# Krabbens/edge-diffusion-tts

Measured on AMD Instinct MI355X. Metric: mel-frames/sec (whole node), 4-step DDIM, hidden=160 L=4, B=256 T=512, higher is better.
Workload: dtype f32

## Files before the change

### edge-diffusion-tts_amd/csrc/edtts_bf16.h

```cpp
typedef __bf16 bf8 __attribute__((ext_vector_type(8)));
typedef __bf16 bf2 __attribute__((ext_vector_type(2)));
typedef float f2v __attribute__((ext_vector_type(2)));

#define EDTTS_MFMA16(a, b, c) __builtin_amdgcn_mfma_f32_16x16x32_bf16((a), (b), (c), 0, 0, 0)

#ifndef EDTTS_STAMP_HEAD
#define EDTTS_STAMP_HEAD 0
#endif
#ifdef EDTTS_STAMPS
#ifndef EDTTS_STAMP_THREAD
#define EDTTS_STAMP_THREAD 0
#endif
#define STAMP16(i) do { if (a.stamps && blockIdx.x == 0 && threadIdx.x == EDTTS_STAMP_THREAD) a.stamps[i] = __builtin_amdgcn_s_memtime(); } while (0)
#define STAMPX16(p, i) do { if ((p) && blockIdx.x == 0 && threadIdx.x == EDTTS_STAMP_THREAD) (p)[i] = __builtin_amdgcn_s_memtime(); } while (0)
#else
#define STAMP16(i) do { } while (0)
#define STAMPX16(p, i) do { } while (0)
#endif

namespace edtts16 {
using namespace edtts;

template <int H_, int HEADS_, int MEL_, int NF_ = 2>
struct Cfg16 {
// ... 627 lines not shown
#pragma unroll
        for (int ft = 0; ft < NF; ++ft) v[ft] = gt[ft] = splat(0.f);
        gemm16_pair<C::KT, false>(ring, hn, v, gt);
        const f4 vb = *reinterpret_cast<const f4*>(params + 32 * j + 4 * g), gb = *reinterpret_cast<const f4*>(params + 32 * j + 16 + 4 * g);
#pragma unroll
        for (int ft = 0; ft < NF; ++ft) {
          v[ft] += vb;
          gt[ft] += gb;
          const f4 e = {fast_exp2(gt[ft][0] * -1.4426950408889634f), fast_exp2(gt[ft][1] * -1.4426950408889634f),
                        fast_exp2(gt[ft][2] * -1.4426950408889634f), fast_exp2(gt[ft][3] * -1.4426950408889634f)};
          const f4 d = e + 1.0f;
          const f4 rc = {__builtin_amdgcn_rcpf(d[0]), __builtin_amdgcn_rcpf(d[1]), __builtin_amdgcn_rcpf(d[2]), __builtin_amdgcn_rcpf(d[3])};
          act[u][ft] = (v[ft] * gt[ft]) * rc;
        }
      }
      bf8 ab[NF];
#pragma unroll
      for (int ft = 0; ft < NF; ++ft) ab[ft] = pack8(act[0][ft], act[1][ft]);
      ktile16<C::HT>(ring, ab, h);
    }
  }
  STAMP16(4);
  if (TAIL == TAIL_QKV) {
    if (valid) {
#pragma unroll
      for (int nt = 0; nt < C::HT; ++nt)
#pragma unroll
        for (int ft = 0; ft < NF; ++ft) stg4(a.h + h_at<C>(tile0, lane, nt, ft), h[nt][ft]);
    }
    bf8 hn[C::KT][NF];
    rms_norm_pack<C>(h, a.n1w, a.cond + (size_t)b * a.cond_bstride + ((size_t)(a.layer + 1) * 2) * 2 * C::H, g, hn);
    qkv_tail16<C>(ring, hn, a, b, m0, lane, valid);
  } else {
    bf8 hn[C::KT][NF];
    layer_norm_pack<C>(h, a.fnw, a.fnb, g, hn);
    for (int p = 0; p < C::MTP; ++p) {
      f4 e[2][NF];
#pragma unroll
      for (int ft = 0; ft < NF; ++ft) e[0][ft] = e[1][ft] = splat(0.f);
      gemm16_pair<C::KT, false>(ring, hn, e[0], e[1]);
#pragma unroll
      for (int u = 0; u < 2; ++u) {
        const int nt = 2 * p + u;
        if (nt >= C::MT) continue;
        const f4 ob = *reinterpret_cast<const f4*>(params + C::UPB_FLOATS + 16 * nt + 4 * g);
#pragma unroll
        for (int ft = 0; ft < NF; ++ft) {
          const int f = m0 + 16 * ft + fq;
          if (f >= a.T || !valid) continue;
          tail_store<TAIL>(a, f, Tb, ((size_t)b * a.T + f) * C::MEL + 16 * nt + 4 * g, e[u][ft] + ob);
        }
      }
    }
  }
  STAMP16(5);
  ring.drain();
  STAMP16(6);
}

}
```

### edge-diffusion-tts_amd/csrc/edtts_coop.h

```cpp
namespace edtts {

template <class C, int W>
struct Coop {
  static constexpr int NF = C::NF, HT = C::HT;
  static constexpr int TILES = 1;
  static constexpr int THREADS = 64 * W;
  static constexpr int O_BYTES = C::HEADS * C::OHEAD_BYTES;
  static constexpr int Q_BYTES = C::WF * C::H * 4;
  static constexpr int ACT_TILES = 2 * HT;
  static constexpr int ACT_BYTES = ACT_TILES * NF * 1024;
  static constexpr int A_BYTES = O_BYTES + Q_BYTES > ACT_BYTES ? O_BYTES + Q_BYTES : ACT_BYTES;
  static constexpr int X_BYTES = HT * NF * 1024;
  static constexpr int TILE_BYTES = A_BYTES + X_BYTES;
  static constexpr int LDS_BYTES = TILES * TILE_BYTES;
  static constexpr bool FITS = LDS_BYTES * (4 / W) <= 160 * 1024;
  static_assert(W == 2 || W == 4, "waves per tile");
};

template <int LK, bool TWO, class FA, class FB>
EDTTS_DEV void co_preload(__amdgpu_buffer_rsrc_t rs, unsigned voff, FA&& fa, FB&& fb, f4 (&ra)[LK], f4 (&rb)[LK]) {
#pragma unroll
  for (int i = 0; i < LK; ++i) {
    ra[i] = bufld4(rs, voff, fa(i));
    if (TWO) rb[i] = bufld4(rs, voff, fb(i));
// ... 251 lines not shown
            if (nt >= HT) continue;
            for (int k = 0; k < nj; ++k) {
              f4 ra[1], rb[1];
              auto one = [&](int) { return (F_FFN + (unsigned)(j0 + k) * 3u * HT + 2u * HT + (unsigned)nt) * 1024u; };
              co_preload<1, false>(rs, voff, one, one, ra, rb);
              co_ktiles<1, NF, 1, false, false>(rs, voff, ra, rb, one, one, one, one, [&](int, int ft) { return act[(k * NF + ft) * 64]; }, NrFull{}, dacc[i], dummy);
            }
          }
        }
      }
    }
#pragma unroll
    for (int i = 0; i < MINE; ++i)
      if (wv + i * W < HT) x_put(wv + i * W, dacc[i]);
  }
  if (TAIL == TAIL_QKV) {
    auto fr = [&](int t, int k) { return (f_tail + (unsigned)((t >> 1) * 2 * HT + 2 * k + (t & 1))) * 1024u; };
    CoGemm<HT, NF, W> gm;
    gm.preload(rs, voff, wv, 3 * HT, fr);
    __syncthreads();
    add_branch();
    if (valid) {
#pragma unroll
      for (int nt = 0; nt < HT; ++nt)
        if (nt % W == wv) {
#pragma unroll
          for (int ft = 0; ft < NF; ++ft) stg4(hp + 16 * nt + (size_t)ft * 16 * H, h[nt][ft]);
        }
    }
    const float* mod = a.cond + (size_t)b * a.cond_bstride + ((size_t)(a.layer + 1) * 2) * 2 * H;
    rms_norm_tile<HT, NF>(h, a.n1w, mod, g, h);
    coop_qkv<C, W>(a, rs, voff, gm, fr, h, wv, lane, b, m0, valid);
  } else {
    __syncthreads();
    add_branch();
    f4 hn[HT][NF];
    layer_norm_tile<HT, NF>(h, a.fnw, a.fnb, g, hn);
    for (int nt = wv; nt < C::MT; nt += W) {
      f4 e[NF], o[NF];
#pragma unroll
      for (int ft = 0; ft < NF; ++ft) e[ft] = o[ft] = splat(0.f);
      f4 fr[HT];
#pragma unroll
      for (int k = 0; k < HT; ++k) fr[k] = bufld4(rs, voff, (f_tail + (unsigned)(nt * HT + k)) * 1024u);
#pragma unroll
      for (int k = 0; k < HT; ++k)
#pragma unroll
        for (int r = 0; r < 4; ++r)
#pragma unroll
          for (int ft = 0; ft < NF; ++ft) {
            if (k & 1) o[ft] = EDTTS_MFMA(fr[k][r], hn[k][ft][r], o[ft]);
            else e[ft] = EDTTS_MFMA(fr[k][r], hn[k][ft][r], e[ft]);
          }
      const f4 ob = ldg4(a.outp_b + 16 * nt + 4 * g);
#pragma unroll
      for (int ft = 0; ft < NF; ++ft) {
        e[ft] += o[ft];
        const int f = m0 + 16 * ft + fq;
        if (!valid || f >= a.T) continue;
        const size_t idx = ((size_t)b * a.T + f) * C::MEL + 16 * nt + 4 * g;
        tail_store<TAIL>(a, f, Tb, idx, e[ft] + ob);
      }
    }
  }
}

template <class C, int TAIL, int W>
__global__ __launch_bounds__(64 * W) void k_layer_co(KArgs a) {
  extern __shared__ __attribute__((aligned(16))) char smem_co[];
  using CO = Coop<C, W>;
  static_assert(CO::FITS, "cooperative tile state must fit the CU's LDS");
  const int lane = threadIdx.x & 63;
  const int wave = __builtin_amdgcn_readfirstlane(threadIdx.x >> 6);
  const int tpu = a.Tp / C::WF, ntiles = a.B * tpu;
  int tile = remap_block(blockIdx.x, gridDim.x) * CO::TILES + wave / W;
  const bool valid = tile < ntiles;
  tile = valid ? tile : ntiles - 1;
  const int b = tile / tpu;
  coop_layer_tile<C, TAIL, W>(a, smem_co + (wave / W) * CO::TILE_BYTES, wave % W, lane, b, (tile - b * tpu) * C::WF, valid);
}

template <class C, int W>
__global__ __launch_bounds__(64 * W) void k_prologue_co(KArgs a) {
  extern __shared__ __attribute__((aligned(16))) char smem_co[];
  constexpr int NF = C::NF, HT = C::HT, MT = C::MT, H = C::H;
  const int lane = threadIdx.x & 63, fq = lane & 15, g = lane >> 4;
  const int wv = __builtin_amdgcn_readfirstlane(threadIdx.x >> 6);
  const int tpu = a.Tp / C::WF, ntiles = a.B * tpu;
  int tile = remap_block(blockIdx.x, gridDim.x);
  const bool valid = tile < ntiles;
  tile = valid ? tile : ntiles - 1;
  const int b = tile / tpu, m0 = (tile - b * tpu) * C::WF;
  const int Tb = utt_len(a.t_len, b, a.T, a.t_dbl);
  f4* const xb = reinterpret_cast<f4*>(smem_co) + lane;
  const __amdgpu_buffer_rsrc_t rs = make_rsrc(a.stream);
  const unsigned voff = (unsigned)lane * 16u;
// ... 43 lines not shown
```

### edge-diffusion-tts_amd/csrc/edtts_generic.h

```cpp
namespace edtts_gen {

enum { EPI_BIAS = 0, EPI_PE = 1, EPI_RESID = 2, EPI_SWIGLU = 3 };

struct GemmArgs {
  const float* X;
  const float* W;
  const float* bias;
  float* Y;
  const float* pe;
  int M, N, K, ldx, ldy, T;
  int vec_x, vec_w, vec_y;
  DropArgs dr;
};
constexpr int kGBM = 64, kGBN = 64, kGBK = 16, kGLd = kGBK + 1;

template <int EPI, bool DROP = false>
__global__ __launch_bounds__(256) void k_gen_gemm(GemmArgs a) {
  __shared__ float xs[kGBM][kGLd];
  __shared__ float ws[kGBN][kGLd];
  const int tid = threadIdx.x, lane = tid & 63, w = tid >> 6, fq = lane & 15, g = lane >> 4;
  const int m0 = blockIdx.x * kGBM;
  const int n0 = blockIdx.y * (EPI == EPI_SWIGLU ? kGBN / 2 : kGBN);
  const int lr = tid >> 2, lk = 4 * (tid & 3);
  int wrow;
// ... 303 lines not shown
    if (a.x0_all) a.x0_all[idx] = v0;
    a.x_prev[idx] = vn;
  } else if (TAIL == TAIL_VLMS) {
    const float v = a.v_uncond ? cfg_combine(e, a.v_uncond[idx], a.vp.cfg) : e;
    const float hn = a.lms.mode >= 2 ? a.h_new[idx] : 0.f, ho = a.lms.mode >= 3 ? a.h_old[idx] : 0.f;
    float v0, vn;
    lms_elem(a.x[idx], v, hn, ho, a.lms, v0, vn);
    a.x0_hist[idx] = v0;
    if (a.x0_all) a.x0_all[idx] = v0;
    if (a.known != nullptr) {
      const size_t row = (size_t)a.T * a.inj_mel, b = idx / row, r = idx - b * row, per = (size_t)a.inj_frames * a.inj_mel;
      if (r < per) {
        const size_t ki = b * per + r;
        vn = a.known[ki];
        if (a.p_coef2 != 0.f) {
          const float nz = a.noise ? a.noise[ki]
                                   : (a.seeds ? philox_normal4(a.seeds[b], a.step, r >> 2)[(int)(r & 3)] : philox_normal4(a.seed, a.step, ki >> 2)[(int)(ki & 3)]);
          vn = qsample_elem(vn, a.p_coef1, nz, a.p_coef2);
        }
      }
    }
    a.x_prev[idx] = vn;
  } else if (TAIL == TAIL_VPRED) {
    const float v = a.v_uncond ? cfg_combine(e, a.v_uncond[idx], a.vp.cfg) : e;
    a.x_prev[idx] = vpred_elem(a.x[idx], v, a.vp);
  } else if (TAIL == TAIL_DDPM) {
    const unsigned long long ge = a.philox_base + idx;
    const float nz = a.noise ? a.noise[idx] : philox_normal4(a.seed, a.step, ge >> 2)[(int)(ge & 3)];
    const DdpmCoef cf{a.p_coef1, a.p_coef2, a.p_sd};
    a.x_prev[idx] = ddpm_elem(a.x[idx], e, nz, cf);
  } else {
    float v0, vp;
    ddim_elem(a.x[idx], e, a.c_s1m, a.c_sab, a.c_sabp, a.c_dir, v0, vp);
    a.x0[idx] = v0;
    a.x_prev[idx] = vp;
  }
}
template <int TAIL>
EDTTS_DEV void tail_zero_elem(const KArgs& a, size_t idx) {
  if (TAIL == TAIL_LMS || TAIL == TAIL_VLMS) {
    a.x0_hist[idx] = 0.f;
    if (a.x0_all) a.x0_all[idx] = 0.f;
  } else if (TAIL == TAIL_DDIM) {
    a.x0[idx] = 0.f;
  }
  a.x_prev[idx] = 0.f;
}
EDTTS_DEV bool past_len(const int64_t* t_len, bool dbl, size_t idx, int T, int MEL) {
  if (t_len == nullptr) return false;
  const size_t row = idx / MEL;
  return (int)(row % T) >= utt_len_lane(t_len, (int)(row / T), T, dbl);
}
template <int TAIL>
__global__ __launch_bounds__(256) void k_gen_tail(KArgs a, const float* eps, size_t n, int vec, int MEL) {
  const size_t stride = (size_t)gridDim.x * blockDim.x;
  if (vec) {
    for (size_t i = (size_t)blockIdx.x * blockDim.x + threadIdx.x; i < n / 4; i += stride) {
      if constexpr (TAIL == TAIL_VLMS) {
        const size_t row = 4 * i / MEL;
        const int f = (int)(row % a.T);
        const int Tb = a.t_len ? utt_len_of(a.t_len[row / a.T], a.T, a.t_dbl) : a.T;
        tail_store<TAIL>(a, f, Tb, 4 * i, ldg4(eps + 4 * i));
        continue;
      }
      if (past_len(a.t_len, a.t_dbl, 4 * i, a.T, MEL)) tail_zero<TAIL>(a, 4 * i);
      else tail_apply<TAIL>(a, 4 * i, ldg4(eps + 4 * i));
    }
  } else {
    for (size_t i = (size_t)blockIdx.x * blockDim.x + threadIdx.x; i < n; i += stride) {
      if (past_len(a.t_len, a.t_dbl, i, a.T, MEL)) tail_zero_elem<TAIL>(a, i);
      else tail_elem<TAIL>(a, i, eps[i]);
    }
  }
}
__global__ __launch_bounds__(256) void k_gen_zero_past(float* y, const int64_t* t_len, int dbl, size_t n, int T, int MEL) {
  for (size_t i = (size_t)blockIdx.x * blockDim.x + threadIdx.x; i < n; i += (size_t)gridDim.x * blockDim.x)
    if (past_len(t_len, dbl, i, T, MEL)) y[i] = 0.f;
// ... 278 lines not shown
```

### edge-diffusion-tts_amd/csrc/edtts_kernels.hip

```cpp
#include <hip/hip_runtime.h>
#include <math.h>
#include <stdarg.h>
#include <stdlib.h>
#include <stdio.h>
#include <string.h>
#include <atomic>
#include <initializer_list>
#include <mutex>
#include <vector>

#include "../../include/edtts.h"
#include "edtts_device.h"

using namespace edtts;

static thread_local char g_err[512] = "";
static int fail(int code, const char* fmt, ...) __attribute__((format(printf, 2, 3)));
static int fail(int code, const char* fmt, ...) {
  va_list ap;
  va_start(ap, fmt);
  vsnprintf(g_err, sizeof(g_err), fmt, ap);
  va_end(ap);
  return code;
}
// ... 579 lines not shown
        for (int r = 0; r < 4; ++r) {
#pragma unroll
          for (int ft = 0; ft < NF; ++ft) h[nt][ft] = EDTTS_MFMA(fa[r], xin[kt][ft][r], h[nt][ft]);
#pragma unroll
          for (int ft = 0; ft < NF; ++ft) h[nt + 1][ft] = EDTTS_MFMA(fb[r], xin[kt][ft][r], h[nt + 1][ft]);
        }
        ring.template refill_after<N>(i);
        ring.template refill_after<N>(i + 1);
      }
    ring.advance(N);
  }
#pragma unroll
  for (int ft = 0; ft < NF; ++ft) {
    int f = m0 + 16 * ft + fq;
    f = f < a.max_pos ? f : a.max_pos - 1;
#pragma unroll
    for (int nt = 0; nt < C::HT; ++nt) h[nt][ft] += ldg4(a.pe + (size_t)f * C::H + 16 * nt + 4 * g);
  }
  {
    float* hp = a.h + ((size_t)b * a.Tp + m0 + fq) * C::H + 4 * g;
#pragma unroll
    for (int nt = 0; nt < C::HT; ++nt)
#pragma unroll
      for (int ft = 0; ft < NF; ++ft) stg4(hp + 16 * nt + (size_t)ft * 16 * C::H, h[nt][ft]);
  }
  f4 hn[C::HT][NF];
  const float* mod = a.cond + (size_t)b * a.cond_bstride;
  rms_norm_tile<C::HT, NF>(h, a.n1w, mod, g, hn);
  qkv_tail<C>(ring, hn, a, b, m0, lane);
}

enum { TAIL_QKV = 0, TAIL_EPS = 1, TAIL_DDIM = 2, TAIL_DDPM = 3, TAIL_LMS = 4, TAIL_VPRED = 5, TAIL_VLMS = 6 };

template <int TAIL>
EDTTS_DEV void tail_apply(const KArgs& a, size_t idx, f4 ev, bool blend = false) {
  if (TAIL == TAIL_EPS) {
    stg4(a.eps + idx, ev);
  } else if (TAIL == TAIL_LMS) {
    const f4 xv = ldg4(a.x + idx);
    f4 hn = splat(0.f), ho = splat(0.f);
    if (a.lms.mode >= 2) hn = ldg4(a.h_new + idx);
    if (a.lms.mode >= 3) ho = ldg4(a.h_old + idx);
    f4 x0, xn;
#pragma unroll
    for (int r = 0; r < 4; ++r) {
      float v0, vn;
      lms_elem(xv[r], ev[r], hn[r], ho[r], a.lms, v0, vn);
      x0[r] = v0;
      xn[r] = vn;
    }
    stg4(a.x0_hist + idx, x0);
    if (a.x0_all) stg4(a.x0_all + idx, x0);
    stg4(a.x_prev + idx, xn);
  } else if (TAIL == TAIL_VLMS) {
    const bool guided = a.v_uncond != nullptr;
    const f4 xv = ldg4(a.x + idx);
    const f4 vu = ldg4((guided ? a.v_uncond : a.x) + idx);
    f4 hn = splat(0.f), ho = splat(0.f);
    if (a.lms.mode >= 2) hn = ldg4(a.h_new + idx);
    if (a.lms.mode >= 3) ho = ldg4(a.h_old + idx);
    f4 x0, xn;
#pragma unroll
    for (int r = 0; r < 4; ++r) {
      const float v = guided ? cfg_combine(ev[r], vu[r], a.vp.cfg) : ev[r];
      float v0, vn;
      lms_elem(xv[r], v, hn[r], ho[r], a.lms, v0, vn);
      x0[r] = v0;
      xn[r] = vn;
    }
    stg4(a.x0_hist + idx, x0);
    if (a.x0_all) stg4(a.x0_all + idx, x0);
    if (!blend) stg4(a.x_prev + idx, xn);
  } else if (TAIL == TAIL_VPRED) {
    const bool guided = a.v_uncond != nullptr;
    const f4 xv = ldg4(a.x + idx);
    const f4 vu = ldg4((guided ? a.v_uncond : a.x) + idx);
    f4 v, xn;
#pragma unroll
    for (int r = 0; r < 4; ++r) v[r] = guided ? cfg_combine(ev[r], vu[r], a.vp.cfg) : ev[r];
#pragma unroll
    for (int r = 0; r < 4; ++r) xn[r] = vpred_elem(xv[r], v[r], a.vp);
    stg4(a.x_prev + idx, xn);
  } else if (TAIL == TAIL_DDPM) {
    const f4 xv = ldg4(a.x + idx);
    const f4 nz = a.noise ? ldg4(a.noise + idx) : philox_normal4(a.seed, a.step, (a.philox_base + idx) >> 2);
    const DdpmCoef cf{a.p_coef1, a.p_coef2, a.p_sd};
    f4 xp;
#pragma unroll
    for (int r = 0; r < 4; ++r) xp[r] = ddpm_elem(xv[r], ev[r], nz[r], cf);
    stg4(a.x_prev + idx, xp);
  } else {
    const f4 xv = ldg4(a.x + idx);
    f4 x0, xp;
#pragma unroll
    for (int r = 0; r < 4; ++r) {
      float v0, vp;
      ddim_elem(xv[r], ev[r], a.c_s1m, a.c_sab, a.c_sabp, a.c_dir, v0, vp);
      x0[r] = v0;
      xp[r] = vp;
    }
    stg4(a.x0 + idx, x0);
    stg4(a.x_prev + idx, xp);
  }
}
template <int TAIL>
EDTTS_DEV void tail_zero(const KArgs& a, size_t idx) {
  const f4 z = splat(0.f);
  if (TAIL == TAIL_EPS) {
    stg4(a.eps + idx, z);
  } else if (TAIL == TAIL_LMS || TAIL == TAIL_VLMS) {
    stg4(a.x0_hist + idx, z);
    if (a.x0_all) stg4(a.x0_all + idx, z);
    stg4(a.x_prev + idx, z);
  } else if (TAIL == TAIL_DDIM) {
    stg4(a.x0 + idx, z);
    stg4(a.x_prev + idx, z);
  } else {
    stg4(a.x_prev + idx, z);
  }
}
EDTTS_DEV void vlms_blend(const KArgs& a, size_t idx) {
  const size_t row = (size_t)a.T * a.inj_mel, b = idx / row, r = idx - b * row;
  const size_t ki = b * ((size_t)a.inj_frames * a.inj_mel) + r;
  const f4 kv = ldg4(a.known + ki);
  f4 o = kv;
  if (a.p_coef2 != 0.f) {
    const unsigned long long sd = a.seeds ? a.seeds[b] : a.seed;
    const f4 nz = a.noise ? ldg4(a.noise + ki) : philox_normal4(sd, a.step, (a.seeds ? r : ki) >> 2);
#pragma unroll
    for (int e = 0; e < 4; ++e) o[e] = qsample_elem(kv[e], a.p_coef1, nz[e], a.p_coef2);
  }
  stg4(a.x_prev + idx, o);
}
template <int TAIL>
EDTTS_DEV void tail_store(const KArgs& a, int f, int Tb, size_t idx, f4 ev) {
  if constexpr (TAIL == TAIL_VLMS) {
    const bool blend = a.known != nullptr && f < Tb && f < a.inj_frames;
    if (f < Tb) tail_apply<TAIL>(a, idx, ev, blend);
    else tail_zero<TAIL>(a, idx);
    if (blend) vlms_blend(a, idx);
  } else {
    if (f < Tb) tail_apply<TAIL>(a, idx, ev);
    else tail_zero<TAIL>(a, idx);
  }
}

struct QGlobal {
  __amdgpu_buffer_rsrc_t rs;
  unsigned v4, v2;
  int H;
  EDTTS_DEV QGlobal(const float* row_m0, int H_, int fq, int g) : rs(make_rsrc(row_m0)), v4((unsigned)(fq * H_ + 4 * g) * 4u), v2((unsigned)(fq * H_ + 2 * g) * 4u), H(H_) {}
  EDTTS_DEV f4 q4(int ft, int col) const { return bufld4(rs, v4, (unsigned)(ft * 16 * H + col) * 4u); }
  EDTTS_DEV f2 q2(int ft, int col) const { return bufld2(rs, v2, (unsigned)(ft * 16 * H + col) * 4u); }
};
struct QLds {
  const float* b4;
  const float* b2;
  int ld;
  EDTTS_DEV QLds(const float* tile, int ld_, int fq, int g) : b4(tile + fq * ld_ + 4 * g), b2(tile + fq * ld_ + 2 * g), ld(ld_) {}
  EDTTS_DEV f4 q4(int ft, int col) const { return *reinterpret_cast<const f4*>(b4 + ft * 16 * ld + col); }
  EDTTS_DEV f2 q2(int ft, int col) const { return *reinterpret_cast<const f2*>(b2 + ft * 16 * ld + col); }
};

template <class C, int TAIL>
EDTTS_DEV void layer_tile(const KArgs& a, float* smem, int wave, int lane, int b, int m0, int Tb, int Sb) {
  constexpr int NF = C::NF;
  const int fq = lane & 15, g = lane >> 4;
  f4* const stash = reinterpret_cast<f4*>(smem) + (size_t)wave * C::HT * NF * 64 + lane;
  constexpr int QLDS = C::H;
  float* qtile = smem + (size_t)C::WAVES * C::HT * NF * 256 + (size_t)wave * C::WF * QLDS;
  const size_t rowbase = (size_t)b * a.Tp + m0 + fq;

  STAMPX(a.stamps, 0, a.diag_skip);
  WStream<C> ring;
  ring.prime(a.stream, lane);

  f4 h[C::HT][NF];
// ... 78 lines not shown
#pragma unroll
    for (int nt = 0; nt < C::HT; ++nt) {
      const f4 db = ldg4(a.down_b + 16 * nt + 4 * g);
#pragma unroll
      for (int ft = 0; ft < NF; ++ft) h[nt][ft] = db;
    }
    for (int j = 0; j < a.ffn_tiles; ++j) {
      const f4 vb = ldg4(a.up_b + 32 * j + 4 * g), gb = ldg4(a.up_b + 32 * j + 16 + 4 * g);
      f4 v[NF], gt[NF], act[NF];
#pragma unroll
      for (int ft = 0; ft < NF; ++ft) v[ft] = gt[ft] = splat(0.f);
      gemm_phase_pair<C::HT>(ring, hn, v, gt);
      __builtin_amdgcn_sched_barrier(0);
#pragma unroll
      for (int ft = 0; ft < NF; ++ft) act[ft] = swiglu_tile(v[ft], gt[ft], vb, gb);
      __builtin_amdgcn_sched_barrier(0);
      ktile_phase<C::HT>(ring, act, h);
    }
    add_parked_h();
    STAMPX(a.stamps, 4, a.diag_skip);
  }
  if (TAIL == TAIL_QKV) {
    {
      float* hp = a.h + rowbase * C::H + 4 * g;
#pragma unroll
      for (int nt = 0; nt < C::HT; ++nt)
#pragma unroll
        for (int ft = 0; ft < NF; ++ft) stg4(hp + 16 * nt + (size_t)ft * 16 * C::H, h[nt][ft]);
    }
    const float* mod = a.cond + (size_t)b * a.cond_bstride + ((size_t)(a.layer + 1) * 2) * 2 * C::H;
    rms_norm_tile<C::HT, NF>(h, a.n1w, mod, g, h);
    qkv_tail<C>(ring, h, a, b, m0, lane);
  } else {
    f4 hn[C::HT][NF];
    layer_norm_tile<C::HT, NF>(h, a.fnw, a.fnb, g, hn);
#pragma unroll
    for (int nt = 0; nt < C::MT; ++nt) {
      const f4 ob = ldg4(a.outp_b + 16 * nt + 4 * g);
      f4 e[NF];
#pragma unroll
      for (int ft = 0; ft < NF; ++ft) e[ft] = splat(0.f);
      gemm_phase<C::HT>(ring, hn, e);
#pragma unroll
      for (int ft = 0; ft < NF; ++ft) {
        const int f = m0 + 16 * ft + fq;
        if (f >= a.T) continue;
        const size_t idx = ((size_t)b * a.T + f) * C::MEL + 16 * nt + 4 * g;
        tail_store<TAIL>(a, f, Tb, idx, e[ft] + ob);
      }
    }
  }
  STAMPX(a.stamps, 5, a.diag_skip);
#ifdef EDTTS_STAMPS
  asm volatile("s_waitcnt vmcnt(0)" ::: "memory");
#endif
  STAMPX(a.stamps, 6, a.diag_skip);
}

template <class C, int TAIL>
EDTTS_DEV void tail_zero_tile(const KArgs& a, int b, int m0, int lane) {
  const int fq = lane & 15, g = lane >> 4;
#pragma unroll
  for (int ft = 0; ft < C::NF; ++ft) {
    const int f = m0 + 16 * ft + fq;
    if (f >= a.T) continue;
#pragma unroll
    for (int nt = 0; nt < C::MT; ++nt) tail_zero<TAIL>(a, ((size_t)b * a.T + f) * C::MEL + 16 * nt + 4 * g);
  }
}
template <class C, int TAIL>
__global__ __launch_bounds__(C::THREADS, 1) void k_layer(KArgs a) {
  extern __shared__ __attribute__((aligned(16))) float smem[];
  const int lane = threadIdx.x & 63;
  const int wave = __builtin_amdgcn_readfirstlane(threadIdx.x >> 6);
  const TileId tl = wave_tile(a.B, a.Tp, C::WAVES, C::WF);
  if (!tl.valid) return;
  const int Tb = utt_len(a.t_len, tl.b, a.T, a.t_dbl);
  if (tl.m0 >= live_end(Tb)) {
    if constexpr (TAIL != TAIL_QKV) tail_zero_tile<C, TAIL>(a, tl.b, tl.m0, lane);
    return;
  }
  const int Sb = utt_len(a.s_len, tl.b, a.S);
// ... 1929 lines not shown
```

### edge-diffusion-tts_amd/csrc/edtts_samplers.h

```cpp

struct StepArgs {
  const float *alphas, *alpha_bar, *betas, *post_var;
  int n_table;
  const float *x, *eps, *noise;
  const int64_t *t, *t_prev;
  size_t n_per_batch;
  float eta;
  float *x_prev, *x0;
  int vec4;
};
static int step_vec4(size_t n_per_batch, std::initializer_list<const void*> ptrs) {
  uintptr_t m = 0;
  for (const void* p : ptrs) m |= (uintptr_t)p;
  return (n_per_batch & 3) == 0 && (m & 15) == 0;
}
EDTTS_DEV long clamp_idx(long v, int n) { return v < 0 ? 0 : (v >= n ? n - 1 : v); }

__global__ __launch_bounds__(256) void k_ddim(StepArgs a) {
  const int b = blockIdx.y;
  const float ab = a.alpha_bar[clamp_idx((long)a.t[b], a.n_table)];
  const long tp = (long)a.t_prev[b];
  const float abp = tp >= 0 ? a.alpha_bar[clamp_idx(tp, a.n_table)] : 1.0f;
  const DdimCoef cf = ddim_coef(ab, abp, a.eta);
  const float s1m = cf.s1m, sab = cf.sab, sabp = cf.sabp, cdir = cf.cdir, sigma = cf.sigma;
// ... 240 lines not shown

static unsigned step_blocks(const StepArgs& a) {
  const size_t bx = ((a.vec4 ? a.n_per_batch / 4 : a.n_per_batch) + 255) / 256;
  return bx > 2048 ? 2048u : (bx < 1 ? 1u : (unsigned)bx);
}

extern "C" {

int edtts_generate(const EdttsDims* dims, const void* packed, void* workspace, int B, int S, const int64_t* sem_idx,
                   const float* x_T, int num_steps, const int64_t* timesteps_host, const float* coef_host, float* x_work,
                   float* x0_out, void* stream) {
  return edtts_generate_len(dims, packed, workspace, B, S, sem_idx, nullptr, x_T, num_steps, timesteps_host, coef_host, x_work, x0_out,
                            stream);
}

int edtts_generate_len(const EdttsDims* dims, const void* packed, void* workspace, int B, int S, const int64_t* sem_idx,
                       const int64_t* s_len, const float* x_T, int num_steps, const int64_t* timesteps_host, const float* coef_host,
                       float* x_work, float* x0_out, void* stream) {
  const SettingsScope settings;
  Layout lo;
  TRY_G(make_layout(dims, &lo));
  if (!packed || !workspace || !sem_idx || !x_T || !timesteps_host || !coef_host || !x_work || !x0_out)
    return fail(EDTTS_ERR_ARG, "NULL pointer argument");
  if (num_steps < 1 || num_steps > lo.NSTEP)
    return fail(EDTTS_ERR_ARG, "num_steps=%d outside [1,%d] (step_emb rows; the reference raises IndexError)", num_steps, lo.NSTEP);
  const int T = 2 * S;
  TRY_G(check_shapes(lo, B, T, S));
  SamplerInputs in;
  in.t_host = timesteps_host; in.sem_idx = sem_idx;
  in.ln = Lens{s_len, s_len, true};
  in.x_T = x_T; in.x = x_work;
  return run_sampler(dims, lo, packed, workspace, B, T, S, num_steps, in, stream, [&](int i, int, size_t o) {
    StepTail tail;
    tail.kind = TAIL_DDIM; tail.x_prev = x_work + o; tail.x0 = x0_out + o; tail.coef = coef_host + 4 * i;
    return tail;
  });
}

int edtts_sample_multistep(const EdttsDims* dims, const void* packed, void* workspace, int B, int T, int S, const int64_t* sem_idx,
                           const float* sem_features, const float* x_T, int num_steps, const int64_t* timesteps_host,
                           const float* coef_host, float* hist, float* x0_all, float* x_out, void* stream) {
  return edtts_sample_multistep_len(dims, packed, workspace, B, T, S, sem_idx, sem_features, nullptr, nullptr, x_T, num_steps,
                                    timesteps_host, coef_host, hist, x0_all, x_out, stream);
}

int edtts_sample_multistep_len(const EdttsDims* dims, const void* packed, void* workspace, int B, int T, int S, const int64_t* sem_idx,
                               const float* sem_features, const int64_t* t_len, const int64_t* s_len, const float* x_T, int num_steps,
                               const int64_t* timesteps_host, const float* coef_host, float* hist, float* x0_all, float* x_out,
                               void* stream) {
  const SettingsScope settings;
  Layout lo;
  TRY_G(make_layout(dims, &lo));
  if (!sem_idx && !sem_features) return fail(EDTTS_ERR_ARG, "Either sem_idx or sem_features must be provided");
  if (!packed || !workspace || !x_T || !timesteps_host || !coef_host || !hist || !x_out) return fail(EDTTS_ERR_ARG, "NULL pointer argument");
  if (num_steps < 1 || num_steps > lo.NSTEP)
    return fail(EDTTS_ERR_ARG, "num_steps=%d outside [1,%d] (step_emb rows; the reference raises IndexError)", num_steps, lo.NSTEP);
  TRY_G(check_shapes(lo, B, T, S));
  TRY_G(check_lms_modes(coef_host, num_steps));
  SamplerInputs in;
  in.t_host = timesteps_host; in.sem_idx = sem_idx; in.sem_features = sem_features;
  in.ln = Lens{t_len, s_len};
  in.x_T = x_T; in.x = x_out;
  const size_t per = (size_t)B * T * lo.MEL;
  return run_sampler(dims, lo, packed, workspace, B, T, S, num_steps, in, stream, [&](int i, int, size_t o) {
    StepTail tail;
    tail.kind = TAIL_LMS; tail.x_prev = x_out + o;
    tail.lms = lms_step_args(coef_host + 8 * i, hist, x0_all, per, i, o);
// ... 177 lines not shown
```

Baseline: 8.746 million.

## Prefetch sampler-tail operands before output GEMM and skip intermediate x0 stores

Splits the fused sampler tail into request/update/commit phases, so loads of x, history, noise and bias for the output projection are issued before the final GEMM and their latency overlaps the MFMA work. Output tiles are grouped by a register-budget heuristic, and stores are batched after all updates. Separately, DDIM generation now writes x0 only on the last step, removing redundant global stores on earlier steps. This raises register pressure and adds scheduling barriers, which could lower occupancy or force spills.

New measurement: 8.723 million. About the same (-0.3%).

```diff
diff --git a/edge-diffusion-tts_amd/csrc/edtts_bf16.h b/edge-diffusion-tts_amd/csrc/edtts_bf16.h
--- a/edge-diffusion-tts_amd/csrc/edtts_bf16.h
+++ b/edge-diffusion-tts_amd/csrc/edtts_bf16.h
@@ -683,25 +683,24 @@
     rms_norm_pack<C>(h, a.n1w, a.cond + (size_t)b * a.cond_bstride + ((size_t)(a.layer + 1) * 2) * 2 * C::H, g, hn);
     qkv_tail16<C>(ring, hn, a, b, m0, lane, valid);
   } else {
+    constexpr int GP = tile_tail_group<NF, TAIL, C::KT * NF * 4, C::MTP, 2>();
+    TileTail<C, TAIL, 2 * GP> tt;
     bf8 hn[C::KT][NF];
     layer_norm_pack<C>(h, a.fnw, a.fnb, g, hn);
-    for (int p = 0; p < C::MTP; ++p) {
-      f4 e[2][NF];
-#pragma unroll
-      for (int ft = 0; ft < NF; ++ft) e[0][ft] = e[1][ft] = splat(0.f);
-      gemm16_pair<C::KT, false>(ring, hn, e[0], e[1]);
-#pragma unroll
-      for (int u = 0; u < 2; ++u) {
-        const int nt = 2 * p + u;
-        if (nt >= C::MT) continue;
-        const f4 ob = *reinterpret_cast<const f4*>(params + C::UPB_FLOATS + 16 * nt + 4 * g);
-#pragma unroll
-        for (int ft = 0; ft < NF; ++ft) {
-          const int f = m0 + 16 * ft + fq;
-          if (f >= a.T || !valid) continue;
-          tail_store<TAIL>(a, f, Tb, ((size_t)b * a.T + f) * C::MEL + 16 * nt + 4 * g, e[u][ft] + ob);
-        }
-      }
+    __builtin_amdgcn_sched_barrier(0);
+    tt.request(a, params + C::UPB_FLOATS, b, m0, Tb, lane, [](int i) { return i < C::MT ? i : -1; });
+#pragma unroll
+    for (int p0 = 0; p0 < C::MTP; p0 += GP) {
+      auto nt_of = [p0](int i) { return 2 * p0 + i < C::MT ? 2 * p0 + i : -1; };
+      if (p0 > 0) tt.request(a, params + C::UPB_FLOATS, b, m0, Tb, lane, nt_of);
+      f4 e[2 * GP][NF];
+#pragma unroll
+      for (int j = 0; j < GP; ++j) {
+#pragma unroll
+        for (int ft = 0; ft < NF; ++ft) e[2 * j][ft] = e[2 * j + 1][ft] = splat(0.f);
+        if (p0 + j < C::MTP) gemm16_pair<C::KT, false>(ring, hn, e[2 * j], e[2 * j + 1]);
+      }
+      tt.finish(a, b, m0, Tb, lane, nt_of, e, valid);
     }
   }
   STAMP16(5);
diff --git a/edge-diffusion-tts_amd/csrc/edtts_coop.h b/edge-diffusion-tts_amd/csrc/edtts_coop.h
--- a/edge-diffusion-tts_amd/csrc/edtts_coop.h
+++ b/edge-diffusion-tts_amd/csrc/edtts_coop.h
@@ -307,14 +307,23 @@
     rms_norm_tile<HT, NF>(h, a.n1w, mod, g, h);
     coop_qkv<C, W>(a, rs, voff, gm, fr, h, wv, lane, b, m0, valid);
   } else {
+    constexpr int MINE = (C::MT + W - 1) / W;
+    auto nt_of = [wv](int i) { return wv + i * W < C::MT ? wv + i * W : -1; };
+    TileTail<C, TAIL, MINE> tt;
     __syncthreads();
     add_branch();
     f4 hn[HT][NF];
     layer_norm_tile<HT, NF>(h, a.fnw, a.fnb, g, hn);
-    for (int nt = wv; nt < C::MT; nt += W) {
+    __builtin_amdgcn_sched_barrier(0);
+    tt.request(a, a.outp_b, b, m0, Tb, lane, nt_of);
+    f4 ev[MINE][NF];
+#pragma unroll
+    for (int i = 0; i < MINE; ++i) {
+      const int nt = nt_of(i);
       f4 e[NF], o[NF];
 #pragma unroll
-      for (int ft = 0; ft < NF; ++ft) e[ft] = o[ft] = splat(0.f);
+      for (int ft = 0; ft < NF; ++ft) ev[i][ft] = e[ft] = o[ft] = splat(0.f);
+      if (nt < 0) continue;
       f4 fr[HT];
 #pragma unroll
       for (int k = 0; k < HT; ++k) fr[k] = bufld4(rs, voff, (f_tail + (unsigned)(nt * HT + k)) * 1024u);
@@ -327,16 +336,10 @@
             if (k & 1) o[ft] = EDTTS_MFMA(fr[k][r], hn[k][ft][r], o[ft]);
             else e[ft] = EDTTS_MFMA(fr[k][r], hn[k][ft][r], e[ft]);
           }
-      const f4 ob = ldg4(a.outp_b + 16 * nt + 4 * g);
-#pragma unroll
-      for (int ft = 0; ft < NF; ++ft) {
-        e[ft] += o[ft];
-        const int f = m0 + 16 * ft + fq;
-        if (!valid || f >= a.T) continue;
-        const size_t idx = ((size_t)b * a.T + f) * C::MEL + 16 * nt + 4 * g;
-        tail_store<TAIL>(a, f, Tb, idx, e[ft] + ob);
-      }
-    }
+#pragma unroll
+      for (int ft = 0; ft < NF; ++ft) ev[i][ft] = e[ft] + o[ft];
+    }
+    tt.finish(a, b, m0, Tb, lane, nt_of, ev, valid);
   }
 }
 
diff --git a/edge-diffusion-tts_amd/csrc/edtts_generic.h b/edge-diffusion-tts_amd/csrc/edtts_generic.h
--- a/edge-diffusion-tts_amd/csrc/edtts_generic.h
+++ b/edge-diffusion-tts_amd/csrc/edtts_generic.h
@@ -359,7 +359,7 @@
   } else {
     float v0, vp;
     ddim_elem(a.x[idx], e, a.c_s1m, a.c_sab, a.c_sabp, a.c_dir, v0, vp);
-    a.x0[idx] = v0;
+    if (a.x0) a.x0[idx] = v0;
     a.x_prev[idx] = vp;
   }
 }
@@ -369,7 +369,7 @@
     a.x0_hist[idx] = 0.f;
     if (a.x0_all) a.x0_all[idx] = 0.f;
   } else if (TAIL == TAIL_DDIM) {
-    a.x0[idx] = 0.f;
+    if (a.x0) a.x0[idx] = 0.f;
   }
   a.x_prev[idx] = 0.f;
 }
diff --git a/edge-diffusion-tts_amd/csrc/edtts_kernels.hip b/edge-diffusion-tts_amd/csrc/edtts_kernels.hip
--- a/edge-diffusion-tts_amd/csrc/edtts_kernels.hip
+++ b/edge-diffusion-tts_amd/csrc/edtts_kernels.hip
@@ -635,117 +635,209 @@
 
 enum { TAIL_QKV = 0, TAIL_EPS = 1, TAIL_DDIM = 2, TAIL_DDPM = 3, TAIL_LMS = 4, TAIL_VPRED = 5, TAIL_VLMS = 6 };
 
+template <int TAIL> constexpr bool tail_is_lms = TAIL == TAIL_LMS || TAIL == TAIL_VLMS;
+template <int TAIL> constexpr bool tail_is_cfg = TAIL == TAIL_VPRED || TAIL == TAIL_VLMS;
+template <int TAIL> constexpr int tail_operands = TAIL == TAIL_EPS ? 0 : TAIL == TAIL_DDIM ? 1 : TAIL == TAIL_LMS ? 3 : TAIL == TAIL_VLMS ? 6 : 2;
+struct TailIn {
+  f4 x;
+  f4 u;
+  f4 hn, ho;
+  f4 nz;
+  f4 kn;
+};
+struct TailOut { f4 a, b; };
 template <int TAIL>
-EDTTS_DEV void tail_apply(const KArgs& a, size_t idx, f4 ev, bool blend = false) {
-  if (TAIL == TAIL_EPS) {
-    stg4(a.eps + idx, ev);
-  } else if (TAIL == TAIL_LMS) {
-    const f4 xv = ldg4(a.x + idx);
-    f4 hn = splat(0.f), ho = splat(0.f);
-    if (a.lms.mode >= 2) hn = ldg4(a.h_new + idx);
-    if (a.lms.mode >= 3) ho = ldg4(a.h_old + idx);
+EDTTS_DEV void tail_request(const KArgs& a, size_t idx, size_t ki, TailIn& o) {
+  if constexpr (TAIL != TAIL_EPS) o.x = ldg4(a.x + idx);
+  if constexpr (tail_is_lms<TAIL>) {
+    o.hn = ldg4((a.lms.mode >= 2 ? a.h_new : a.x) + idx);
+    o.ho = ldg4((a.lms.mode >= 3 ? a.h_old : a.x) + idx);
+  }
+  if constexpr (tail_is_cfg<TAIL>) o.u = ldg4((a.v_uncond != nullptr ? a.v_uncond : a.x) + idx);
+  if constexpr (TAIL == TAIL_DDPM) o.nz = ldg4((a.noise != nullptr ? a.noise : a.x) + idx);
+  if constexpr (TAIL == TAIL_VLMS) {
+    const bool kn = a.known != nullptr;
+    o.kn = ldg4(kn ? a.known + ki : a.x + idx);
+    o.nz = ldg4(kn && a.noise != nullptr ? a.noise + ki : a.x + idx);
+  }
+}
+EDTTS_DEV unsigned long long blend_seed(const KArgs& a, size_t kb) { return a.seeds ? a.seeds[kb] : a.seed; }
+template <int TAIL>
+EDTTS_DEV void tail_update(const KArgs& a, size_t idx, f4 ev, const TailIn& in, bool live, TailOut& out, bool blend = false, size_t kb = 0,
+                           size_t kr = 0, unsigned long long sd = 0) {
+  const f4 z = splat(0.f);
+  if constexpr (TAIL == TAIL_EPS) {
+    out.a = live ? ev : z;
+  } else if constexpr (tail_is_lms<TAIL>) {
+    const bool guided = TAIL == TAIL_VLMS && a.v_uncond != nullptr;
+    const f4 hn = a.lms.mode >= 2 ? in.hn : z, ho = a.lms.mode >= 3 ? in.ho : z;
     f4 x0, xn;
 #pragma unroll
     for (int r = 0; r < 4; ++r) {
+      float v = ev[r];
+      if constexpr (TAIL == TAIL_VLMS) v = guided ? cfg_combine(ev[r], in.u[r], a.vp.cfg) : ev[r];
       float v0, vn;
-      lms_elem(xv[r], ev[r], hn[r], ho[r], a.lms, v0, vn);
+      lms_elem(in.x[r], v, hn[r], ho[r], a.lms, v0, vn);
       x0[r] = v0;
       xn[r] = vn;
     }
-    stg4(a.x0_hist + idx, x0);
-    if (a.x0_all) stg4(a.x0_all + idx, x0);
-    stg4(a.x_prev + idx, xn);
-  } else if (TAIL == TAIL_VLMS) {
+    out.a = live ? x0 : z;
+    out.b = live ? xn : z;
+    if constexpr (TAIL == TAIL_VLMS) {
+      if (a.known != nullptr) {
+        f4 o = in.kn;
+        if (a.p_coef2 != 0.f) {
+          const size_t ki = kb * ((size_t)a.inj_frames * a.inj_mel) + kr;
+          const f4 nz = a.noise ? in.nz : philox_normal4(sd, a.step, (a.seeds ? kr : ki) >> 2);
+#pragma unroll
+          for (int e = 0; e < 4; ++e) o[e] = qsample_elem(in.kn[e], a.p_coef1, nz[e], a.p_coef2);
+        }
+        out.b = blend ? o : out.b;
+      }
+    }
+  } else if constexpr (TAIL == TAIL_VPRED) {
     const bool guided = a.v_uncond != nullptr;
-    const f4 xv = ldg4(a.x + idx);
-    const f4 vu = ldg4((guided ? a.v_uncond : a.x) + idx);
-    f4 hn = splat(0.f), ho = splat(0.f);
-    if (a.lms.mode >= 2) hn = ldg4(a.h_new + idx);
-    if (a.lms.mode >= 3) ho = ldg4(a.h_old + idx);
-    f4 x0, xn;
-#pragma unroll
-    for (int r = 0; r < 4; ++r) {
-      const float v = guided ? cfg_combine(ev[r], vu[r], a.vp.cfg) : ev[r];
-      float v0, vn;
-      lms_elem(xv[r], v, hn[r], ho[r], a.lms, v0, vn);
-      x0[r] = v0;
-      xn[r] = vn;
-    }
-    stg4(a.x0_hist + idx, x0);
-    if (a.x0_all) stg4(a.x0_all + idx, x0);
-    if (!blend) stg4(a.x_prev + idx, xn);
-  } else if (TAIL == TAIL_VPRED) {
-    const bool guided = a.v_uncond != nullptr;
-    const f4 xv = ldg4(a.x + idx);
-    const f4 vu = ldg4((guided ? a.v_uncond : a.x) + idx);
     f4 v, xn;
 #pragma unroll
-    for (int r = 0; r < 4; ++r) v[r] = guided ? cfg_combine(ev[r], vu[r], a.vp.cfg) : ev[r];
-#pragma unroll
-    for (int r = 0; r < 4; ++r) xn[r] = vpred_elem(xv[r], v[r], a.vp);
-    stg4(a.x_prev + idx, xn);
-  } else if (TAIL == TAIL_DDPM) {
-    const f4 xv = ldg4(a.x + idx);
-    const f4 nz = a.noise ? ldg4(a.noise + idx) : philox_normal4(a.seed, a.step, (a.philox_base + idx) >> 2);
+    for (int r = 0; r < 4; ++r) v[r] = guided ? cfg_combine(ev[r], in.u[r], a.vp.cfg) : ev[r];
+#pragma unroll
+    for (int r = 0; r < 4; ++r) xn[r] = vpred_elem(in.x[r], v[r], a.vp);
+    out.a = live ? xn : z;
+  } else if constexpr (TAIL == TAIL_DDPM) {
+    const f4 nz = a.noise ? in.nz : philox_normal4(a.seed, a.step, (a.philox_base + idx) >> 2);
     const DdpmCoef cf{a.p_coef1, a.p_coef2, a.p_sd};
     f4 xp;
 #pragma unroll
-    for (int r = 0; r < 4; ++r) xp[r] = ddpm_elem(xv[r], ev[r], nz[r], cf);
-    stg4(a.x_prev + idx, xp);
+    for (int r = 0; r < 4; ++r) xp[r] = ddpm_elem(in.x[r], ev[r], nz[r], cf);
+    out.a = live ? xp : z;
   } else {
-    const f4 xv = ldg4(a.x + idx);
     f4 x0, xp;
 #pragma unroll
     for (int r = 0; r < 4; ++r) {
       float v0, vp;
-      ddim_elem(xv[r], ev[r], a.c_s1m, a.c_sab, a.c_sabp, a.c_dir, v0, vp);
+      ddim_elem(in.x[r], ev[r], a.c_s1m, a.c_sab, a.c_sabp, a.c_dir, v0, vp);
       x0[r] = v0;
       xp[r] = vp;
     }
-    stg4(a.x0 + idx, x0);
-    stg4(a.x_prev + idx, xp);
-  }
+    out.a = live ? x0 : z;
+    out.b = live ? xp : z;
+  }
+}
+template <int TAIL>
+EDTTS_DEV void tail_commit(const KArgs& a, size_t idx, const TailOut& o) {
+  if constexpr (TAIL == TAIL_EPS) {
+    stg4(a.eps + idx, o.a);
+  } else if constexpr (tail_is_lms<TAIL>) {
+    stg4(a.x0_hist + idx, o.a);
+    if (a.x0_all) stg4(a.x0_all + idx, o.a);
+    stg4(a.x_prev + idx, o.b);
+  } else if constexpr (TAIL == TAIL_DDIM) {
+    if (a.x0) stg4(a.x0 + idx, o.a);
+    stg4(a.x_prev + idx, o.b);
+  } else {
+    stg4(a.x_prev + idx, o.a);
+  }
+}
+template <int TAIL>
+EDTTS_DEV void tail_apply(const KArgs& a, size_t idx, f4 ev) {
+  TailIn in;
+  TailOut o;
+  tail_request<TAIL>(a, idx, 0, in);
+  tail_update<TAIL>(a, idx, ev, in, true, o);
+  tail_commit<TAIL>(a, idx, o);
 }
 template <int TAIL>
 EDTTS_DEV void tail_zero(const KArgs& a, size_t idx) {
-  const f4 z = splat(0.f);
-  if (TAIL == TAIL_EPS) {
-    stg4(a.eps + idx, z);
-  } else if (TAIL == TAIL_LMS || TAIL == TAIL_VLMS) {
-    stg4(a.x0_hist + idx, z);
-    if (a.x0_all) stg4(a.x0_all + idx, z);
-    stg4(a.x_prev + idx, z);
-  } else if (TAIL == TAIL_DDIM) {
-    stg4(a.x0 + idx, z);
-    stg4(a.x_prev + idx, z);
-  } else {
-    stg4(a.x_prev + idx, z);
-  }
-}
-EDTTS_DEV void vlms_blend(const KArgs& a, size_t idx) {
-  const size_t row = (size_t)a.T * a.inj_mel, b = idx / row, r = idx - b * row;
-  const size_t ki = b * ((size_t)a.inj_frames * a.inj_mel) + r;
-  const f4 kv = ldg4(a.known + ki);
-  f4 o = kv;
-  if (a.p_coef2 != 0.f) {
-    const unsigned long long sd = a.seeds ? a.seeds[b] : a.seed;
-    const f4 nz = a.noise ? ldg4(a.noise + ki) : philox_normal4(sd, a.step, (a.seeds ? r : ki) >> 2);
-#pragma unroll
-    for (int e = 0; e < 4; ++e) o[e] = qsample_elem(kv[e], a.p_coef1, nz[e], a.p_coef2);
-  }
-  stg4(a.x_prev + idx, o);
+  TailOut o;
+  o.a = o.b = splat(0.f);
+  tail_commit<TAIL>(a, idx, o);
 }
 template <int TAIL>
 EDTTS_DEV void tail_store(const KArgs& a, int f, int Tb, size_t idx, f4 ev) {
+  if (f >= Tb) return tail_zero<TAIL>(a, idx);
   if constexpr (TAIL == TAIL_VLMS) {
-    const bool blend = a.known != nullptr && f < Tb && f < a.inj_frames;
-    if (f < Tb) tail_apply<TAIL>(a, idx, ev, blend);
-    else tail_zero<TAIL>(a, idx);
-    if (blend) vlms_blend(a, idx);
+    const bool blend = a.known != nullptr && f < a.inj_frames;
+    const size_t row = (size_t)a.T * a.inj_mel, kb = blend ? idx / row : 0, kr = blend ? idx - kb * row : 0;
+    TailIn in;
+    TailOut o;
+    tail_request<TAIL>(a, idx, blend ? kb * ((size_t)a.inj_frames * a.inj_mel) + kr : 0, in);
+    tail_update<TAIL>(a, idx, ev, in, true, o, blend, kb, kr, blend ? blend_seed(a, kb) : 0);
+    tail_commit<TAIL>(a, idx, o);
   } else {
-    if (f < Tb) tail_apply<TAIL>(a, idx, ev);
-    else tail_zero<TAIL>(a, idx);
-  }
+    tail_apply<TAIL>(a, idx, ev);
+  }
+}
+
+template <class C, int TAIL, int N>
+struct TileTail {
+  TailIn in[N][C::NF];
+  f4 ob[N];
+  unsigned long long sd;
+  static EDTTS_DEV int slot(int nt) { return nt < 0 ? 0 : nt; }
+  template <class NtOf>
+  EDTTS_DEV void request(const KArgs& a, const float* outp_b, int b, int m0, int Tb, int lane, NtOf&& nt_of) {
+    const int fq = lane & 15, g = lane >> 4;
+    sd = 0;
+    if constexpr (TAIL == TAIL_VLMS) {
+      if (a.known != nullptr) sd = blend_seed(a, (size_t)__builtin_amdgcn_readfirstlane(b));
+    }
+#pragma unroll
+    for (int i = 0; i < N; ++i) ob[i] = ldg4(outp_b + 16 * slot(nt_of(i)) + 4 * g);
+#pragma unroll
+    for (int ft = 0; ft < C::NF; ++ft) {
+      const int f = m0 + 16 * ft + fq, fc = f < Tb ? f : Tb - 1;
+      const size_t row = ((size_t)b * a.T + fc) * C::MEL + 4 * g;
+      size_t krow = 0;
+      if constexpr (TAIL == TAIL_VLMS) {
+        const int fk = fc < a.inj_frames ? fc : (a.inj_frames > 0 ? a.inj_frames - 1 : 0);
+        krow = ((size_t)b * a.inj_frames + fk) * C::MEL + 4 * g;
+      }
+#pragma unroll
+      for (int i = 0; i < N; ++i) tail_request<TAIL>(a, row + 16 * slot(nt_of(i)), krow + 16 * slot(nt_of(i)), in[i][ft]);
+    }
+    __builtin_amdgcn_sched_barrier(0);
+  }
+  template <class NtOf>
+  EDTTS_DEV void finish(const KArgs& a, int b, int m0, int Tb, int lane, NtOf&& nt_of, const f4 (&e)[N][C::NF], bool store) {
+    const int fq = lane & 15, g = lane >> 4;
+    TailOut out[N][C::NF];
+    __builtin_amdgcn_sched_barrier(0);
+#pragma unroll
+    for (int ft = 0; ft < C::NF; ++ft) {
+      const int f = m0 + 16 * ft + fq;
+      const size_t row = ((size_t)b * a.T + f) * C::MEL + 4 * g;
+      const bool live = f < Tb, blend = TAIL == TAIL_VLMS && live && f < a.inj_frames;
+#pragma unroll
+      for (int i = 0; i < N; ++i)
+        tail_update<TAIL>(a, row + 16 * slot(nt_of(i)), e[i][ft] + ob[i], in[i][ft], live, out[i][ft], blend, (size_t)b,
+                          (size_t)f * C::MEL + 16 * slot(nt_of(i)) + 4 * g, sd);
+    }
+#pragma unroll
+    for (int ft = 0; ft < C::NF; ++ft)
+#pragma unroll
+      for (int i = 0; i < N; ++i) {
+        asm volatile("" : "+v"(out[i][ft].a));
+        if constexpr (TAIL == TAIL_DDIM || tail_is_lms<TAIL>) asm volatile("" : "+v"(out[i][ft].b));
+      }
+    __builtin_amdgcn_sched_barrier(0);
+#pragma unroll
+    for (int ft = 0; ft < C::NF; ++ft) {
+      const int f = m0 + 16 * ft + fq;
+      if (f >= a.T || !store) continue;
+      const size_t row = ((size_t)b * a.T + f) * C::MEL + 4 * g;
+#pragma unroll
+      for (int i = 0; i < N; ++i)
+        if (nt_of(i) >= 0) tail_commit<TAIL>(a, row + 16 * nt_of(i), out[i][ft]);
+    }
+  }
+};
+template <int NF, int TAIL, int FIXED_REGS, int UNITS, int TILES_PER_UNIT = 1>
+constexpr int tile_tail_group() {
+  constexpr int per_unit = TILES_PER_UNIT * ((tail_operands<TAIL> + 3) * 4 * NF + 4);
+  constexpr int room = 416 - FIXED_REGS;
+  int groups = 1;
+  while ((UNITS + groups - 1) / groups * per_unit > room && groups < UNITS) ++groups;
+  return (UNITS + groups - 1) / groups;
 }
 
 struct QGlobal {
@@ -890,22 +982,24 @@
     rms_norm_tile<C::HT, NF>(h, a.n1w, mod, g, h);
     qkv_tail<C>(ring, h, a, b, m0, lane);
   } else {
+    constexpr int GN = tile_tail_group<NF, TAIL, (C::HT * NF + WStream<C>::RN_) * 4, C::MT>();
+    TileTail<C, TAIL, GN> tt;
     f4 hn[C::HT][NF];
     layer_norm_tile<C::HT, NF>(h, a.fnw, a.fnb, g, hn);
-#pragma unroll
-    for (int nt = 0; nt < C::MT; ++nt) {
-      const f4 ob = ldg4(a.outp_b + 16 * nt + 4 * g);
-      f4 e[NF];
-#pragma unroll
-      for (int ft = 0; ft < NF; ++ft) e[ft] = splat(0.f);
-      gemm_phase<C::HT>(ring, hn, e);
-#pragma unroll
-      for (int ft = 0; ft < NF; ++ft) {
-        const int f = m0 + 16 * ft + fq;
-        if (f >= a.T) continue;
-        const size_t idx = ((size_t)b * a.T + f) * C::MEL + 16 * nt + 4 * g;
-        tail_store<TAIL>(a, f, Tb, idx, e[ft] + ob);
-      }
+    __builtin_amdgcn_sched_barrier(0);
+    tt.request(a, a.outp_b, b, m0, Tb, lane, [](int i) { return i < C::MT ? i : -1; });
+#pragma unroll
+    for (int n0 = 0; n0 < C::MT; n0 += GN) {
+      auto nt_of = [n0](int i) { return n0 + i < C::MT ? n0 + i : -1; };
+      if (n0 > 0) tt.request(a, a.outp_b, b, m0, Tb, lane, nt_of);
+      f4 e[GN][NF];
+#pragma unroll
+      for (int i = 0; i < GN; ++i) {
+#pragma unroll
+        for (int ft = 0; ft < NF; ++ft) e[i][ft] = splat(0.f);
+        if (n0 + i < C::MT) gemm_phase<C::HT>(ring, hn, e[i]);
+      }
+      tt.finish(a, b, m0, Tb, lane, nt_of, e, true);
     }
   }
   STAMPX(a.stamps, 5, a.diag_skip);
diff --git a/edge-diffusion-tts_amd/csrc/edtts_samplers.h b/edge-diffusion-tts_amd/csrc/edtts_samplers.h
--- a/edge-diffusion-tts_amd/csrc/edtts_samplers.h
+++ b/edge-diffusion-tts_amd/csrc/edtts_samplers.h
@@ -296,7 +296,7 @@
   in.x_T = x_T; in.x = x_work;
   return run_sampler(dims, lo, packed, workspace, B, T, S, num_steps, in, stream, [&](int i, int, size_t o) {
     StepTail tail;
-    tail.kind = TAIL_DDIM; tail.x_prev = x_work + o; tail.x0 = x0_out + o; tail.coef = coef_host + 4 * i;
+    tail.kind = TAIL_DDIM; tail.x_prev = x_work + o; tail.x0 = i == num_steps - 1 ? x0_out + o : nullptr; tail.coef = coef_host + 4 * i;
     return tail;
   });
 }
```
